# cliarie/radix-join

Measured on AMD Instinct MI355X. Metric: probe_tuples_per_sec, higher is better.
Workload: dtype int32

## Files before the change

### include/rj.h

```cpp
#ifndef RJ_H_
#define RJ_H_

#include <stddef.h>
#include <stdint.h>

#ifdef __cplusplus
extern "C" {
#endif

#define RJ_PAGE_SIZE 8192u

typedef enum rj_dtype {
    RJ_INT32   = 0,
    RJ_INT64   = 1,
    RJ_FP64    = 2,
    RJ_VARCHAR = 3
} rj_dtype;

typedef enum rj_status {
    RJ_OK            = 0,
    RJ_ERR_ARG       = 1,
    RJ_ERR_DEVICE    = 2,
    RJ_ERR_NOMEM     = 3,
    RJ_ERR_DATA      = 4,
// ... 243 lines not shown
    uint64_t bins;
} rj_partition_pass;
typedef struct rj_partition_plan {
    uint32_t passes;
    uint32_t pbits[RJ_PLAN_MAX_PASSES];
    int32_t  fine, fine_xcd;
    uint32_t fine_grid;
    int32_t  mid, last;
    int32_t  spec, spec2;
    uint64_t spec_cap_max, spec2_cap_max;
    uint64_t n_first_out, n_last_out;
    uint32_t tpg_first, reserved;
    rj_partition_pass pass[RJ_PLAN_MAX_PASSES];
} rj_partition_plan;
int rj_debug_partition_plan(const rj_partition_request* req, uint32_t compute_units, rj_partition_plan* out);
uint64_t rj_table_num_rows(const rj_table* t);
uint64_t rj_table_col_pages(const rj_table* t, uint64_t col);
int      rj_table_copy_pages(rj_context* ctx, const rj_table* t, uint64_t col, void* const* dst, uint64_t n_dst);

typedef struct rj_result rj_result;

enum { RJ_EXEC_KEEP_ON_DEVICE = 1 };

int rj_execute(rj_context* ctx, const rj_plan* plan, rj_result** out);
int rj_execute_resident(rj_context* ctx, const rj_plan* plan, rj_table* const* tables,
                        uint64_t n_tables, int32_t flags, rj_result** out);

uint64_t rj_result_num_rows(const rj_result* r);
uint64_t rj_result_num_cols(const rj_result* r);
int32_t  rj_result_col_type(const rj_result* r, uint64_t col);
// ... 58 lines not shown
```

### radix-join_amd/csrc/rj_api.hip

```cpp
#include <chrono>
#include <cstdlib>
#include <mutex>

#include "rj_frame.hpp"
#include "rj_fsum.hpp"
#include "rj_internal.hpp"
#include "rj_radix_plan.hpp"
#include "rj_sortkey.hpp"
#include "rj_xplan.hpp"

using namespace rj;

static std::mutex  g_err_mu;
static std::string g_create_error;

template <class F>
static int guarded(rj_context* ctx, F&& f) {
    try {
        f();
        return RJ_OK;
    } catch (const rj::Error& e) {
        if (ctx) ctx->last_error = e.what();
        return e.code;
    } catch (const std::bad_alloc&) {
// ... 191 lines not shown
    *n_out = 0;
    try {
        rj::map_eval_row(ops, n_ops, n_cols, col_type, col_bits, col_null, out_cap, out_bits, out_null, out_kind, n_out);
        return RJ_OK;
    } catch (const rj::Error& e) {
        std::lock_guard<std::mutex> g(g_err_mu);
        g_create_error = e.what();
        return e.code;
    } catch (const std::exception& e) {
        std::lock_guard<std::mutex> g(g_err_mu);
        g_create_error = e.what();
        return RJ_ERR_DEVICE;
    }
}

int rj_debug_partition_plan(const rj_partition_request* req, uint32_t compute_units, rj_partition_plan* out) {
    if (!req || !out) return RJ_ERR_ARG;
    if (req->key_words < 1 || req->key_words > 2 || req->carry_words < 0 || req->key_words + req->carry_words > MAX_WORDS) return RJ_ERR_ARG;
    if (req->bits > 32 || (req->single_pass && req->bits > (uint32_t)PT_MAXBITS)) return RJ_ERR_ARG;
    if (req->word_source < 0 || req->word_source > 2 || (req->word_source == 2 && (req->key_words != 1 || req->carry_words != 1))) return RJ_ERR_ARG;
    RadixFacts f;
    f.n = req->n;
    f.KW = req->key_words, f.CW = req->carry_words, f.bits = req->bits, f.shift0 = req->shift0;
    f.single_pass = req->single_pass != 0;
    f.word_src = req->word_source != 0, f.word_src_packed = req->word_source == 2;
    f.external = req->external != 0, f.composite = req->composite != 0;
    f.preseg_nseg = req->preseg_nseg, f.preseg_n_oseg = req->preseg_n_oseg;
    f.after_offsets = req->after_offsets != 0, f.spec_flag = req->flag_word != 0, f.spec2_ok = req->spec2_ok != 0;
    Tuning tune;
    tune.from_env();
    const RadixPlan pl = radix_plan(f, tune, (int)compute_units);
    static_assert((int)RadixMid::Aos3Side == RJ_MID_AOS3_SIDE && (int)RadixLast::Aos3 == RJ_LAST_AOS3 &&
                      (int)RadixOffsets::Chunked == RJ_OFF_CHUNKED && (int)RadixHist::LastSample == RJ_HIST_LAST_SAMPLE &&
                      (int)RadixScatter::LastDense == RJ_SCATTER_LAST_DENSE,
                  "include/rj.h lists the plan's enums in the order of rj_radix_plan.hpp");
    *out = rj_partition_plan{};
    out->passes = pl.passes();
    out->fine = pl.fine, out->fine_xcd = pl.fine_xcd, out->fine_grid = pl.fine_grid;
    out->mid = (int32_t)pl.mid, out->last = (int32_t)pl.last;
    out->spec = pl.spec, out->spec2 = pl.spec2;
    out->spec_cap_max = pl.spec_cap_max, out->spec2_cap_max = pl.spec2_cap_max;
    out->n_first_out = pl.n_first_out, out->n_last_out = pl.n_last_out;
    out->tpg_first = pl.tpg_first;
    for (uint32_t p = 0; p < pl.passes() && p < RJ_PLAN_MAX_PASSES; ++p) {
        const RadixPass&   ps = pl.pass[p];
        rj_partition_pass& o = out->pass[p];
        out->pbits[p] = pl.pbits[p];
        o.bits = ps.bits, o.tiles_per_group = ps.tiles_per_group, o.xcd_log2 = ps.xcd_log2, o.xcd_remap = ps.xcd_remap;
        o.nseg_in = ps.nseg_in, o.n_oseg = ps.n_oseg, o.n_groups = ps.n_groups, o.bins = ps.bins;
        o.offsets = (int32_t)ps.offsets, o.hist = (int32_t)ps.hist, o.scatter = (int32_t)ps.scatter;
    }
    return RJ_OK;
}

int rj_debug_launch_log(rj_context* ctx, int on) {
    if (!ctx) return RJ_ERR_ARG;
    for (int l = 0; l < ctx->n_lanes(); ++l) {
        ctx->lane(l)->klog.clear();
        ctx->lane(l)->klog.on = on != 0;
    }
    return RJ_OK;
}

int rj_debug_launch_read(rj_context* ctx, char* buf, uint64_t cap, uint64_t* need) {
    if (!ctx || !need || (cap && !buf)) return RJ_ERR_ARG;
    return guarded(ctx, [&] {
// ... 275 lines not shown
```

### radix-join_amd/csrc/rj_context.hip

```cpp
#include <dlfcn.h>

#include <algorithm>
#include <chrono>
#include <cstdlib>

#include "rj_internal.hpp"

namespace rj {

[[noreturn]] void launch_failed(const char* kernel, const char* what, bool unsupported) {
    throw_fmt(unsupported ? RJ_ERR_UNSUPPORTED : RJ_ERR_DEVICE, "launch %s: %s", kernel, what);
}

static int env_int(const char* name, int def) {
    const char* v = getenv(name);
    return v && *v ? atoi(v) : def;
}

void Tuning::from_env() {
    blocked_mid = env_int("RJ_TUNE_BLOCKED_MID", blocked_mid);
    mall_chunk = env_int("RJ_TUNE_MALL_CHUNK", mall_chunk);
    radix_bits = env_int("RJ_TUNE_RADIX_BITS", radix_bits);
    p1_bits = env_int("RJ_TUNE_P1_BITS", p1_bits);
    fine = env_int("RJ_TUNE_FINE", fine);
// ... 1 lines not shown
    aos3 = env_int("RJ_TUNE_AOS3", aos3);
    aos_mid = env_int("RJ_TUNE_AOS_MID", aos_mid);
    tpg1 = env_int("RJ_TUNE_TPG1", tpg1);
    xcd_split = env_int("RJ_TUNE_XCD_SPLIT", xcd_split);
    tpg2 = env_int("RJ_TUNE_TPG2", tpg2);
    packed_side = env_int("RJ_TUNE_PACKED_SIDE", packed_side);
    xcd_min_rows = env_int("RJ_TUNE_XCD_MIN_ROWS", xcd_min_rows);
    spec_p1 = env_int("RJ_TUNE_SPEC_P1", spec_p1);
    spec_min_rows = env_int("RJ_TUNE_SPEC_MIN_ROWS", spec_min_rows);
    spec_sample = std::min(5, std::max(1, env_int("RJ_TUNE_SPEC_SAMPLE", spec_sample)));
    spec_z = std::max(0, env_int("RJ_TUNE_SPEC_Z", spec_z));
    spec_p2 = env_int("RJ_TUNE_SPEC_P2", spec_p2);
    spec2_min_rows = env_int("RJ_TUNE_SPEC2_MIN_ROWS", spec2_min_rows);
    spec2_sample = std::min(4, std::max(1, env_int("RJ_TUNE_SPEC2_SAMPLE", spec2_sample)));
    spec2_z = std::max(0, env_int("RJ_TUNE_SPEC2_Z", spec2_z));
    bcast = env_int("RJ_TUNE_BCAST", bcast);
    diag = env_int("RJ_DIAG", diag);
    varchar_dev_rows = env_int("RJ_TUNE_VARCHAR_DEV", varchar_dev_rows);
    vkey_hash_bits = env_int("RJ_DEBUG_VKEY_HASH_BITS", vkey_hash_bits);
    sync_upload = env_int("RJ_SYNC_UPLOAD", sync_upload);
    wide_carry = env_int("RJ_TUNE_WIDE_CARRY", wide_carry);
    fold_owner = env_int("RJ_TUNE_FOLD_OWNER", fold_owner);
    group_grid = env_int("RJ_TUNE_GROUP_GRID", group_grid);
    win_grid = env_int("RJ_TUNE_WIN_GRID", win_grid);
    map_grid = env_int("RJ_TUNE_MAP_GRID", map_grid);
    setop_grid = env_int("RJ_TUNE_SETOP_GRID", setop_grid);
    exchange_timeout_ms = env_int("RJ_EXCHANGE_TIMEOUT_MS", exchange_timeout_ms);
    bringup_timeout_ms = env_int("RJ_BRINGUP_TIMEOUT_MS", bringup_timeout_ms);
    debug_shard_fail = env_int("RJ_DEBUG_SHARD_FAIL", debug_shard_fail);
    debug_shard_fail_rank = env_int("RJ_DEBUG_SHARD_FAIL_RANK", debug_shard_fail_rank);
// ... 299 lines not shown
```

### radix-join_amd/csrc/rj_exec.hip

```cpp
#include <algorithm>
#include <chrono>
#include <cmath>
#include <cstdlib>
#include <functional>
#include <set>
#include <tuple>

#include "rj_expr.hpp"
#include "rj_internal.hpp"
#include "rj_radix.hpp"
#include "rj_xplan.hpp"

namespace rj {

const NodeKind* node_kind(int kind) {
    static const NodeKind kinds[] = {
        {RJ_NODE_SCAN, "a scan", "RJ_NODE_SCAN", 0, true},
        {RJ_NODE_JOIN, "a join", "RJ_NODE_JOIN", 2, true},
        {RJ_NODE_SEMI, "a semi join", "RJ_NODE_SEMI", 2, false},
        {RJ_NODE_ANTI, "an anti join", "RJ_NODE_ANTI", 2, false},
        {RJ_NODE_OUTER, "an outer join", "RJ_NODE_OUTER", 2, false},
        {RJ_NODE_FULL, "a full outer join", "RJ_NODE_FULL", 2, false},
        {RJ_NODE_AGG, "an aggregation", "RJ_NODE_AGG", 1, false},
        {RJ_NODE_SELECT, "a selection", "RJ_NODE_SELECT", 1, false},
// ... 584 lines not shown
    }

    struct CoParts {
        Parted   B, P;
        BufP     tasks;
        uint32_t max_tasks = 0;
    };
    CoParts partition_sides(JoinState& st, const JoinSpec& js, uint32_t bits, const BufP* counters = nullptr, bool spec2_ok = false) {
        CoParts        cp;
        const TupleSrc sb = make_src(st, st.bs(), js), sp = make_src(st, st.ps(), js);
        uint32_t*      fl = counters ? (*counters)->as<uint32_t>() + 4 : nullptr;
        PartitionRequest rb = PartitionRequest::columns(sb, st.KW, st.bs().CW, bits), rp = PartitionRequest::columns(sp, st.KW, st.ps().CW, bits);
        rb.spec_flag = fl;
        rp.spec_flag = fl ? fl + 1 : nullptr;
        rb.spec2_ok = rp.spec2_ok = spec2_ok;
        cp.B = partition(rb);
        cp.P = partition(rp);
        return cp;
    }
    int  spec_fallbacks = 0;
    void repartition_exact(JoinState& st, const JoinSpec& js, uint32_t bits, CoParts& cp, const BufP& counters, bool flag_b,
                           bool flag_p) {
        ++spec_fallbacks;
        if (ctx->tune.diag >= 1)
            fprintf(stderr, "[rj diag] %s: a speculative pass overflowed (build side %d, probe side %d): exact partition again (fallback %d of this plan)\n",
                    st.kind->name, (int)flag_b, (int)flag_p, spec_fallbacks);
        if (flag_b) {
            const TupleSrc sb = make_src(st, st.bs(), js);
            cp.B = Parted();
            cp.B = partition(PartitionRequest::columns(sb, st.KW, st.bs().CW, bits));
        }
        if (flag_p) {
// ... 2445 lines not shown
```

### radix-join_amd/csrc/rj_internal.hpp

```cpp
#pragma once
#include <hip/hip_runtime.h>

#include <atomic>
#include <cstdarg>
#include <cstdio>
#include <cstring>
#include <functional>
#include <map>
#include <memory>
#include <mutex>
#include <stdexcept>
#include <string>
#include <vector>

#include "../../include/rj.h"
#include "rj_comm.hpp"
#include "rj_device.hpp"
#include "rj_kernels.hpp"

namespace rj {

struct Context;

struct Error : std::runtime_error {
// ... 153 lines not shown
    int aos3 = 1;
    int aos_mid = 2;
    int tpg1 = 0;
    int packed_side = 0;
    int tpg2 = 0;
    int xcd_min_rows = 40 << 20;
    int xcd_split = 1;
    int spec_p1 = 1;
    int spec_min_rows = 40 << 20;
    int spec_sample = 5;
    int spec_z = 60;
    int spec_p2 = 1;
    int spec2_min_rows = 40 << 20;
    int spec2_sample = 2;
    int spec2_z = 70;
    int bcast = 1;
    int diag = 0;
    int varchar_dev_rows = 200000;
    int vkey_hash_bits = 0;
    int sync_upload = 0;
    int wide_carry = 1;
    int fold_owner = 1;
    int group_grid = 0;
    int map_grid = 0;
    int win_grid = 0;
    int setop_grid = 0;
    int exchange_timeout_ms = 120000;
    int bringup_timeout_ms = 0;
    int debug_shard_fail = 0, debug_shard_fail_rank = 0;
    int debug_poison = 0;
// ... 129 lines not shown
```

### radix-join_amd/csrc/rj_radix.hip

```cpp
#include "rj_radix.hpp"

#include <algorithm>

#include "rj_radix_plan.hpp"

namespace rj {

void read_back(Context* ctx, void* dst, const void* src, size_t bytes) {
    try {
        RJ_HIP(hipMemcpyAsync(dst, src, bytes, hipMemcpyDeviceToHost, ctx->stream));
        ctx->sync();
    } catch (...) {
        (void)hipStreamSynchronize(ctx->stream);
        throw;
    }
}

namespace {

RadixFacts facts_of(const PartitionRequest& rq) {
    RadixFacts f;
    f.n = rq.ws ? rq.ws->n : (rq.src ? rq.src->n_rows : 0);
    f.KW = rq.KW, f.CW = rq.CW, f.bits = rq.bits, f.shift0 = rq.shift0, f.single_pass = rq.single_pass;
    f.word_src = rq.ws != nullptr, f.word_src_packed = rq.ws && rq.ws->packed;
// ... 36 lines not shown
    PassParams       pp{};
    SpecParams       sp{};
    LastParams       lp{};
    BufP             grp_start, off, hist, cursor;
    const uint32_t*  in_end = nullptr;
    const uint32_t*  oseg_base = nullptr;
    PassRun(const RadixPass& s, uint32_t pass) : ps(s), p(pass), F(1u << s.bits) {}
};

class Driver {
   public:
    Driver(Context* c, const Launch& l, const PartitionRequest& r)
        : ctx(c), L(l), rq(r), src(r.src ? *r.src : none), n(r.ws ? r.ws->n : src.n_rows),
          pl(radix_plan(facts_of(r), c->tune, c->compute_units())), passes(pl.passes()) {}

    Parted run() {
        P.NW = rq.KW + rq.CW;
        P.packed = pl.packed(), P.aos3 = pl.aos3(), P.spec = pl.spec, P.spec2 = pl.spec2;
        allocate();
        shift = rq.shift0;
        cur = rq.ws ? rq.ws->w : Words{};
        nxt = (pl.aos3() && passes == 1) ? waos : wa;
        for (uint32_t p = 0; p < passes; ++p) {
            PassRun r(pl.pass[p], p);
            begin_pass(r);
            offsets_for_pass(r);
            if (p == 0 && rq.after_offsets) (*rq.after_offsets)(r.off->as<uint32_t>());
            if (p == 0 && pl.chunk_second()) send_sizes_to_host(r);
            if (r.ps.offsets != RadixOffsets::Chunked) scatter_pass(r);
            advance(r);
        }
        P.w = cur;
        for (int a = 0; a < P.NW; ++a) P.wbuf[a] = cur_is_a ? A[a] : B[a];
        if (pl.aos3()) P.wbuf[0] = AOS;
        P.off = seg_off;
        P.NP = nseg;
        P.pbits = pl.pbits;
        const PassShape* shape = rq.shape;
        if (shape && !shape->prior_bits.empty()) P.pbits.insert(P.pbits.begin(), shape->prior_bits.begin(), shape->prior_bits.end());
        P.n_tuples = n;
        return std::move(P);
    }

   private:
    Context*                ctx;
    const Launch&           L;
    const PartitionRequest& rq;
    const TupleSrc          none{};
    const TupleSrc&         src;
    const uint64_t          n;
    const RadixPlan         pl;
    const uint32_t          passes;
    Parted                  P;
    BufP  A[MAX_WORDS], B[MAX_WORDS], AOS, MID[2], SIDE[2];
    Words wa{}, wb{}, waos{};
    BufP  fine_off, fine_cursor, coarse_off, coarse_cursor;
    BufP  last_limit, last_seg_sum, last_grp;
    BufP  spec_start, spec_limit, spec_end;
    Event chunk_ev;
    BufP     seg_off;
    uint32_t nseg = 1, shift = 0;
    Words    cur{}, nxt{};
    bool     cur_is_a = false;

    void allocate() {
        const uint32_t mids = std::min<uint32_t>(passes - 1, 2);
        if (pl.aos_mid())
            for (uint32_t k = 0; k < mids; ++k) {
                MID[k] = ctx->buf(std::max<uint64_t>(n, 1) * 12);
                if (pl.mid == RadixMid::Aos3Side) SIDE[k] = ctx->buf(std::max<uint64_t>(n, 1) * 2 + 16);
            }
        if (pl.mid == RadixMid::PackedSide)
            for (uint32_t k = 0; k < mids; ++k) SIDE[k] = ctx->buf(std::max<uint64_t>(n, 1) * 2 + 16);
        if (pl.aos3()) {
            AOS = ctx->buf(std::max<uint64_t>(pl.n_last_out, 1) * 12);
            waos.w[0] = AOS->as<uint32_t>();
        }
        for (int a = 0; a < (pl.packed() ? 1 : P.NW); ++a) {
            if (pl.pair_word >= 0 && a == pl.pair_word + 1) continue;
            const uint64_t wbytes = (pl.packed() || a == pl.pair_word) ? 8 : 4;
            if (rq.external) {
                wa.w[a] = rq.external->w[a];
                continue;
            }
            if ((pl.aos3() && passes == 1) || pl.aos_mid()) continue;
            A[a] = ctx->buf(pl.n_first_out * wbytes + 2048);
            wa.w[a] = A[a]->as<uint32_t>();
            if (passes > (pl.aos3() ? 2u : 1u)) {
                B[a] = ctx->buf(pl.n_last_out * wbytes + 2048);
                wb.w[a] = B[a]->as<uint32_t>();
            }
        }
    }

    void begin_pass(PassRun& r) {
        const RadixPass& ps = r.ps;
        const PassShape* shape = r.p == 0 ? rq.shape : nullptr;
        const bool       preseg = shape && shape->nseg > 0;
        PassParams&      pp = r.pp;
        pp.nseg = nseg;
        pp.n = (uint32_t)n;
        pp.shift = shift;
        pp.fanout_log2 = ps.bits;
        pp.tiles_per_group = ps.tiles_per_group;
        pp.xcd_log2 = ps.xcd_log2;
        pp.xcd_remap = ps.xcd_remap;
        if (shape && shape->hi_shift) {
            pp.hi_shift = shape->hi_shift;
            pp.lo_bits = shape->lo_bits;
        }
        r.in_end = preseg ? shape->seg_end : (ps.spec_in ? spec_end->as<uint32_t>() : nullptr);
        r.oseg_base = preseg ? shape->oseg_off : (seg_off ? seg_off->as<uint32_t>() : nullptr);
        if (r.p == 0 && !preseg) return;
        const uint32_t* in_off = preseg ? shape->seg_begin : (ps.spec_in ? spec_start->as<uint32_t>() : seg_off->as<uint32_t>());
        r.grp_start = ctx->buf(((uint64_t)ps.nseg_in + 1) * 4);
        launch_group_table(L, in_off, ps.nseg_in, ps.tiles_per_group * (uint32_t)PT_TILE, r.grp_start->as<uint32_t>(), r.in_end);
        pp.nseg = ps.nseg_in;
        pp.seg_off = in_off;
        pp.seg_end = r.in_end;
        pp.oseg_shift = preseg ? shape->oseg_shift : (ps.spec_in ? 3u : 0u);
        pp.grp_start = r.grp_start->as<uint32_t>();
    }

    void offsets_for_pass(PassRun& r) {
        switch (r.ps.offsets) {
        case RadixOffsets::Fine:
            if (r.ps.hist != RadixHist::None) fine_histogram();
            r.off = r.p == 0 ? coarse_off : fine_off;
            r.cursor = r.p == 0 ? coarse_cursor : fine_cursor;
            r.pp.cursor = r.cursor->as<uint32_t>();
// ... 55 lines not shown
        const uint32_t G = r.ps.n_groups, prev = (r.p + 1) % 2;
        switch (r.ps.hist) {
        case RadixHist::Src: launch_pass_hist_src(L, src, rq.KW, r.pp, G); break;
        case RadixHist::Digits: launch_pass_hist_digits(L, SIDE[prev]->as<uint16_t>(), r.pp, G); break;
        case RadixHist::Aos3: launch_pass_hist_aos3(L, MID[prev]->as<uint32_t>(), r.pp, G); break;
        case RadixHist::Blocked: launch_pass_hist_blocked(L, cur.w[0], r.pp, G); break;
        case RadixHist::Packed: launch_pass_hist_packed(L, cur.w[0], r.pp, G); break;
        case RadixHist::Dense: launch_pass_hist_dense(L, cur, r.pp, G); break;
        default: throw_fmt(RJ_ERR_DEVICE, "radix plan: pass %u has no exact histogram", r.p);
        }
    }

    void sample_first(PassRun& r) {
        const uint32_t spec_s = (uint32_t)ctx->tune.spec_sample;
        const uint32_t nb = (uint32_t)r.ps.bins << 3;
        r.hist = ctx->buf((uint64_t)nb * 4);
        r.off = ctx->buf((r.ps.bins + 1) * 4);
        r.cursor = ctx->buf((uint64_t)nb * 8);
        spec_start = ctx->buf((uint64_t)nb * 4);
        spec_limit = ctx->buf((uint64_t)nb * 4);
        spec_end = ctx->buf((uint64_t)nb * 4);
        RJ_HIP(hipMemsetAsync(r.hist->p, 0, (uint64_t)nb * 4, ctx->stream));
        r.pp.hist = r.hist->as<uint32_t>();
        r.sp.cursor = r.cursor->as<unsigned long long>();
        r.sp.flag = rq.spec_flag;
        r.sp.sink = (uint32_t)pl.spec_cap_max;
        r.sp.sample_log2 = spec_s;
        launch_pass_sample_src(L, src, rq.KW, r.pp, r.sp, r.ps.n_groups);
        launch_spec_caps(L, r.pp.hist, nb, spec_s, (float)(ctx->tune.spec_z / 10.0), (uint32_t)pl.spec_cap_max,
                         spec_start->as<uint32_t>(), spec_limit->as<uint32_t>(), r.sp.cursor);
    }

    void sample_last(PassRun& r) {
        const uint32_t spec2_s = (uint32_t)ctx->tune.spec2_sample;
        const uint32_t nb = (uint32_t)r.ps.bins, nseg_in = r.ps.nseg_in;
        r.hist = ctx->buf((uint64_t)nb * 4);
        r.off = ctx->buf((uint64_t)nb * 8);
        r.cursor = ctx->buf((uint64_t)nb * 4);
        last_limit = ctx->buf((uint64_t)nb * 4);
        last_seg_sum = ctx->buf((uint64_t)r.ps.n_oseg * 8);
        RJ_HIP(hipMemsetAsync(r.hist->p, 0, (uint64_t)nb * 4, ctx->stream));
        r.pp.hist = r.hist->as<uint32_t>();
        r.lp.cursor32 = r.cursor->as<uint32_t>();
        r.lp.limit = last_limit->as<uint32_t>();
        r.lp.flag = rq.spec_flag;
        r.lp.sink = (uint32_t)pl.spec2_cap_max;
        r.lp.sample_log2 = spec2_s;
        PassParams ps = r.pp;
        ps.tiles_per_group = LAST_SAMPLE_TPG;
        last_grp = ctx->buf(((uint64_t)nseg_in + 1) * 4);
        launch_group_table(L, r.pp.seg_off, nseg_in, LAST_SAMPLE_TPG * (uint32_t)PT_TILE, last_grp->as<uint32_t>(), r.in_end);
        ps.grp_start = last_grp->as<uint32_t>();
        launch_last_sample(L, cur.w[0], P.packed, ps, r.lp, r.ps.sample_groups);
        launch_last_caps(L, r.pp.hist, r.ps.n_oseg, r.F, spec2_s, (float)(ctx->tune.spec2_z / 10.0), (uint32_t)pl.spec2_cap_max,
                         last_seg_sum->as<unsigned long long>(), r.off->as<uint32_t>(), last_limit->as<uint32_t>(), r.lp.cursor32);
    }

    void send_sizes_to_host(PassRun& r) {
        const uint64_t bytes = (r.ps.bins + 1) * 4;
        if (bytes > Context::SMALL_PINNED / 4) throw_fmt(RJ_ERR_DEVICE, "chunked pass: too many segments");
        RJ_HIP(hipMemcpyAsync(ctx->small_pinned(), r.off->p, bytes, hipMemcpyDeviceToHost, ctx->stream));
        chunk_ev.make();
        RJ_HIP(hipEventRecord(chunk_ev.e, ctx->stream));
    }

// ... 47 lines not shown
            pp.side_out = SIDE[p % 2]->as<uint16_t>();
            pp.next_shift = shift + ps.bits;
            pp.next_mask = (1u << pl.pbits[p + 1]) - 1u;
        }
        const SpecParams* sp = (p == 0 && pl.spec) ? &r.sp : nullptr;
        switch (ps.scatter) {
        case RadixScatter::Src: launch_pass_scatter_src(L, src, rq.KW, rq.CW, pp, G, nxt, ps.aos_out, sp); break;
        case RadixScatter::SrcPacked: launch_pass_scatter_src_packed(L, src, pp, G, nxt.w[0], ps.blocked_out, sp); break;
        case RadixScatter::Dense: launch_pass_scatter_dense(L, cur, P.NW, pl.pair_word, pp, G, nxt, ps.aos_out); break;
        case RadixScatter::Packed: launch_pass_scatter_packed(L, cur.w[0], pp, G, nxt.w[0]); break;
        case RadixScatter::Blocked: launch_pass_scatter_blocked(L, cur.w[0], pp, G, nxt.w[0], ps.blocked_out); break;
        case RadixScatter::Aos3: launch_pass_scatter_aos3(L, MID[(p + 1) % 2]->as<uint32_t>(), pp, G, nxt.w[0]); break;
        case RadixScatter::LastBlocked: launch_last_scatter_blocked(L, cur.w[0], pp, G, nxt.w[0], r.lp); break;
        case RadixScatter::LastDense: launch_last_scatter_dense(L, cur, pp, G, nxt, r.lp); break;
        }
        const uint32_t bins = (uint32_t)ps.bins;
        if (ps.hist == RadixHist::LastSample) {
            launch_last_close(L, r.lp.cursor32, last_limit->as<uint32_t>(), bins, r.off->as<uint32_t>());
            if (ctx->tune.diag >= 1) spec_report(ctx, r.cursor, last_limit, r.off, bins, n, pl.n_last_out, 2);
            P.off_shift = 1;
        }
        if (ps.hist == RadixHist::SampleSrc) {
            launch_spec_close(L, r.sp.cursor, spec_start->as<uint32_t>(), spec_limit->as<uint32_t>(), r.F, spec_end->as<uint32_t>(),
                              r.off->as<uint32_t>());
            if (ctx->tune.diag >= 1) spec_report(ctx, r.cursor, spec_limit, spec_start, bins << 3, n, pl.n_first_out, 1);
        }
    }

    void advance(PassRun& r) {
        seg_off = r.off;
        nseg = (uint32_t)r.ps.bins;
        shift += r.ps.bits;
        cur = nxt;
        cur_is_a = (r.p % 2 == 0);
        nxt = cur_is_a ? wb : wa;
        if (pl.aos3() && r.p + 2 == passes) nxt = waos;
    }
};

}

Parted radix_partition(Context* ctx, const Launch& L, const PartitionRequest& rq) { return Driver(ctx, L, rq).run(); }

}
```

### radix-join_amd/csrc/rj_radix.hpp

```cpp
#pragma once
#include <functional>

#include "rj_internal.hpp"

namespace rj {

struct Parted {
    int      NW = 0;
    BufP     wbuf[MAX_WORDS];
    Words    w{};
    BufP     off;
    uint32_t NP = 0;
    std::vector<uint32_t> pbits;
    bool     packed = false;
    bool     aos3 = false;
    uint64_t n_tuples = 0;
    bool     spec = false;
    uint32_t off_shift = 0;
    bool     spec2 = false;
};

struct WordSrc {
    Words    w{};
    uint64_t n = 0;
// ... 26 lines not shown

    static PartitionRequest columns(const TupleSrc& s, int KW, int CW, uint32_t bits) {
        PartitionRequest rq;
        rq.src = &s, rq.KW = KW, rq.CW = CW, rq.bits = bits;
        return rq;
    }
    static PartitionRequest words(const WordSrc& s, int KW, int CW, uint32_t bits) {
        PartitionRequest rq;
        rq.ws = &s, rq.KW = KW, rq.CW = CW, rq.bits = bits;
        return rq;
    }
};

Parted radix_partition(Context* ctx, const Launch& L, const PartitionRequest& rq);

struct Event {
    hipEvent_t e = nullptr;
    Event() = default;
    Event(const Event&) = delete;
    Event& operator=(const Event&) = delete;
    void make() { RJ_HIP(hipEventCreateWithFlags(&e, hipEventDisableTiming)); }
    ~Event() {
        if (e) (void)hipEventDestroy(e);
    }
};

void read_back(Context* ctx, void* dst, const void* src, size_t bytes);

}
```

### radix-join_amd/csrc/rj_radix_plan.cpp

```cpp
#include "rj_radix_plan.hpp"

#include <algorithm>
#include <cmath>

#include "rj_internal.hpp"

namespace rj {

uint32_t radix_tiles_per_group(uint64_t tuples_per_segment, uint64_t target_groups) {
    uint64_t k = (tuples_per_segment + (uint64_t)PT_TILE * target_groups - 1) / ((uint64_t)PT_TILE * target_groups);
    return (uint32_t)std::min<uint64_t>(std::max<uint64_t>(k, 1), 8);
}

uint64_t radix_cap_bound(double B, double C, uint32_t s, double z) {
    const double bound = std::ldexp(C + z * std::sqrt(B * (C + B)) + 0.5 * z * z * B, (int)s) + 32.0 * B;
    return bound < 4.0e9 ? (((uint64_t)std::ceil(bound) + 255u) & ~(uint64_t)255u) : ~(uint64_t)0 >> 1;
}

namespace {

void choose_layout(const RadixFacts& f, const Tuning& t, int compute_units, RadixPlan& pl) {
    const uint64_t n = f.n;
    const uint32_t passes = pl.passes(), bits = f.bits;
    const bool     shaped = f.composite || f.preseg_nseg > 0;
// ... 112 lines not shown
        if (b1 < f.bits && b1 <= PT_CAPBITS && f.bits - b1 <= PT_CAPBITS) {
            pl.pbits[0] = b1;
            pl.pbits[1] = f.bits - b1;
        }
    }
    pl.pass.resize(passes);
    choose_layout(f, t, compute_units, pl);
    uint32_t nseg = 1;
    for (uint32_t p = 0; p < passes; ++p) {
        plan_pass(f, t, pl, p, nseg, pl.pass[p]);
        nseg = (uint32_t)pl.pass[p].bins;
    }
    return pl;
}

}
```

### radix-join_amd/csrc/rj_radix_plan.hpp

```cpp
#pragma once
#include <cstdint>
#include <vector>

namespace rj {

struct Tuning;

struct RadixFacts {
    uint64_t n = 0;
    int      KW = 1, CW = 0;
    uint32_t bits = 0, shift0 = 0;
    bool     single_pass = false;
    bool     word_src = false, word_src_packed = false;
    bool     external = false;
    bool     composite = false;
    uint32_t preseg_nseg = 0, preseg_n_oseg = 0;
    bool     after_offsets = false;
    bool     spec_flag = false, spec2_ok = false;
};

enum class RadixMid : int32_t {
    Dense = 0,
    Packed = 1,
    PackedSide = 2,
// ... 41 lines not shown
    bool packed() const { return last == RadixLast::Packed; }
    bool aos3() const { return last == RadixLast::Aos3; }
    bool aos_mid() const { return mid == RadixMid::Aos3 || mid == RadixMid::Aos3Side; }
    bool side() const { return mid == RadixMid::Aos3Side || mid == RadixMid::PackedSide; }
    bool chunk_second() const { return pass.size() == 2 && pass[1].offsets == RadixOffsets::Chunked; }
};

constexpr uint32_t LAST_SAMPLE_TPG = 8;

uint32_t radix_tiles_per_group(uint64_t tuples_per_segment, uint64_t target_groups);

uint64_t radix_cap_bound(double B, double C, uint32_t s, double z);

RadixPlan radix_plan(const RadixFacts& f, const Tuning& tune, int compute_units);

}
```

### radix-join_amd/pyrj/capi.py

```python
from __future__ import annotations

import ctypes as C
import os

import numpy as np

from . import pages as pg
from . import plan as pl

PKG_DIR = os.path.dirname(os.path.dirname(os.path.abspath(__file__)))
LIB_PATH = os.path.join(PKG_DIR, "librj.so")

RJ_EXEC_KEEP_ON_DEVICE = 1


class rj_comm_id(C.Structure):
    _fields_ = [("bytes", C.c_char * 128)]


class rj_config(C.Structure):
    _fields_ = [
        ("device", C.c_int32),
        ("profile", C.c_int32),
        ("stream", C.c_void_p),
# ... 115 lines not shown
    "rj_comm_id_create",
    "rj_execute_sharded",
    "rj_plan_shardable",
    "rj_table_upload",
    "rj_table_adopt_device",
    "rj_table_release",
    "rj_table_from_csv",
    "rj_debug_parse_fp64",
    "rj_debug_sort_key",
    "rj_debug_sort_key_value",
    "rj_debug_win_frame",
    "rj_debug_win_ntile",
    "rj_debug_fsum",
    "rj_debug_map_eval",
    "rj_debug_partition_plan",
    "rj_table_num_rows",
    "rj_table_col_pages",
    "rj_table_copy_pages",
    "rj_execute",
    "rj_execute_resident",
    "rj_result_num_rows",
    "rj_result_num_cols",
    "rj_result_col_type",
    "rj_result_col_pages",
    "rj_result_copy_pages",
    "rj_result_device_pages",
    "rj_result_free",
    "rj_exchange_plan",
    "rj_shard_partition",
    "rj_join_tuples",
# ... 521 lines not shown
                ("reserved", C.c_uint32), ("pass_", rj_partition_pass * 4)]


PLAN_MID = ["dense", "packed", "packed_side", "blocked", "aos3", "aos3_side"]
PLAN_LAST = ["dense", "packed", "aos3"]
PLAN_OFFSETS = ["fine", "hist", "sample", "chunked"]
PLAN_HIST = ["none", "fine_src", "fine_words", "src", "digits", "aos3", "blocked", "packed", "dense", "sample_src", "last_sample"]
PLAN_SCATTER = ["src", "src_packed", "dense", "packed", "blocked", "aos3", "last_blocked", "last_dense"]


def partition_plan(n, kw=1, cw=1, bits=0, *, cus=256, shift0=0, single_pass=False, word_source=0, external=False, composite=False,
                   preseg=(0, 0), after_offsets=False, flag_word=False, spec2_ok=False) -> dict:
    L = load()
    L.rj_debug_partition_plan.restype = C.c_int
    L.rj_debug_partition_plan.argtypes = [C.POINTER(rj_partition_request), C.c_uint32, C.POINTER(rj_partition_plan)]
    rq = rj_partition_request(int(n), kw, cw, bits, shift0, int(single_pass), int(word_source), int(external), int(composite),
                              preseg[0], preseg[1], int(after_offsets), int(flag_word), int(spec2_ok))
    out = rj_partition_plan()
    rc = L.rj_debug_partition_plan(C.byref(rq), cus, C.byref(out))
    if rc != 0:
        raise RjError(rc, "rj_debug_partition_plan: bad request")
    d = {k: int(getattr(out, k)) for k in ("passes", "fine_grid", "spec_cap_max", "spec2_cap_max", "n_first_out", "n_last_out", "tpg_first")}
    d.update({k: bool(getattr(out, k)) for k in ("fine", "fine_xcd", "spec", "spec2")})
    d["pbits"] = [int(out.pbits[p]) for p in range(d["passes"])]
    d["mid"], d["last"] = PLAN_MID[out.mid], PLAN_LAST[out.last]
    d["pass"] = []
    for p in range(d["passes"]):
        ps = out.pass_[p]
        e = {k: int(getattr(ps, k)) for k in ("bits", "tiles_per_group", "xcd_log2", "xcd_remap", "nseg_in", "n_oseg", "n_groups", "bins")}
        e["offsets"], e["hist"], e["scatter"] = PLAN_OFFSETS[ps.offsets], PLAN_HIST[ps.hist], PLAN_SCATTER[ps.scatter]
        d["pass"].append(e)
    return d


def make_comm_id() -> bytes:
    L = load()
    preload_torch_rccl()
    cid = rj_comm_id()
    rc = L.rj_comm_id_create(C.byref(cid))
    if rc != 0:
        raise RjError(rc, (L.rj_last_error(None) or b"").decode())
    return C.string_at(C.addressof(cid), 128)


def build_context(**kw):
    return Context(**kw)


def destroy_context(ctx: Context):
# ... 6 lines not shown
```

Measured before the change: 35.04 billion.

## Interleave build and probe radix partition passes across two streams

```diff
diff --git a/include/rj.h b/include/rj.h
--- a/include/rj.h
+++ b/include/rj.h
@@ -281,6 +281,19 @@
     rj_partition_pass pass[RJ_PLAN_MAX_PASSES];
 } rj_partition_plan;
 int rj_debug_partition_plan(const rj_partition_request* req, uint32_t compute_units, rj_partition_plan* out);
+typedef enum rj_lane_kind { RJ_LANE_OFFSETS = 0, RJ_LANE_SCATTER = 1, RJ_LANE_CLOSE = 2, RJ_LANE_JOIN = 3 } rj_lane_kind;
+typedef struct rj_lane_step {
+    int32_t  side;
+    uint32_t pass;
+    int32_t  kind;
+    int32_t  lane;
+} rj_lane_step;
+typedef struct rj_lane_edge {
+    uint32_t after, before;
+} rj_lane_edge;
+int rj_debug_lane_schedule(const rj_partition_request* build, const rj_partition_request* probe, uint32_t compute_units,
+                           int32_t mask, rj_lane_step* steps, uint64_t step_cap, uint64_t* n_steps, rj_lane_edge* edges,
+                           uint64_t edge_cap, uint64_t* n_edges);
 uint64_t rj_table_num_rows(const rj_table* t);
 uint64_t rj_table_col_pages(const rj_table* t, uint64_t col);
 int      rj_table_copy_pages(rj_context* ctx, const rj_table* t, uint64_t col, void* const* dst, uint64_t n_dst);
diff --git a/radix-join_amd/csrc/rj_api.hip b/radix-join_amd/csrc/rj_api.hip
--- a/radix-join_amd/csrc/rj_api.hip
+++ b/radix-join_amd/csrc/rj_api.hip
@@ -229,12 +229,11 @@
     }
 }
 
-int rj_debug_partition_plan(const rj_partition_request* req, uint32_t compute_units, rj_partition_plan* out) {
-    if (!req || !out) return RJ_ERR_ARG;
-    if (req->key_words < 1 || req->key_words > 2 || req->carry_words < 0 || req->key_words + req->carry_words > MAX_WORDS) return RJ_ERR_ARG;
-    if (req->bits > 32 || (req->single_pass && req->bits > (uint32_t)PT_MAXBITS)) return RJ_ERR_ARG;
-    if (req->word_source < 0 || req->word_source > 2 || (req->word_source == 2 && (req->key_words != 1 || req->carry_words != 1))) return RJ_ERR_ARG;
-    RadixFacts f;
+static bool facts_of_request(const rj_partition_request* req, RadixFacts& f) {
+    if (!req) return false;
+    if (req->key_words < 1 || req->key_words > 2 || req->carry_words < 0 || req->key_words + req->carry_words > MAX_WORDS) return false;
+    if (req->bits > 32 || (req->single_pass && req->bits > (uint32_t)PT_MAXBITS)) return false;
+    if (req->word_source < 0 || req->word_source > 2 || (req->word_source == 2 && (req->key_words != 1 || req->carry_words != 1))) return false;
     f.n = req->n;
     f.KW = req->key_words, f.CW = req->carry_words, f.bits = req->bits, f.shift0 = req->shift0;
     f.single_pass = req->single_pass != 0;
@@ -242,6 +241,12 @@
     f.external = req->external != 0, f.composite = req->composite != 0;
     f.preseg_nseg = req->preseg_nseg, f.preseg_n_oseg = req->preseg_n_oseg;
     f.after_offsets = req->after_offsets != 0, f.spec_flag = req->flag_word != 0, f.spec2_ok = req->spec2_ok != 0;
+    return true;
+}
+
+int rj_debug_partition_plan(const rj_partition_request* req, uint32_t compute_units, rj_partition_plan* out) {
+    RadixFacts f;
+    if (!out || !facts_of_request(req, f)) return RJ_ERR_ARG;
     Tuning tune;
     tune.from_env();
     const RadixPlan pl = radix_plan(f, tune, (int)compute_units);
@@ -265,6 +270,24 @@
         o.nseg_in = ps.nseg_in, o.n_oseg = ps.n_oseg, o.n_groups = ps.n_groups, o.bins = ps.bins;
         o.offsets = (int32_t)ps.offsets, o.hist = (int32_t)ps.hist, o.scatter = (int32_t)ps.scatter;
     }
+    return RJ_OK;
+}
+
+int rj_debug_lane_schedule(const rj_partition_request* build, const rj_partition_request* probe, uint32_t compute_units, int32_t mask,
+                           rj_lane_step* steps, uint64_t step_cap, uint64_t* n_steps, rj_lane_edge* edges, uint64_t edge_cap,
+                           uint64_t* n_edges) {
+    RadixFacts fb, fp;
+    if (!n_steps || !n_edges || (step_cap && !steps) || (edge_cap && !edges)) return RJ_ERR_ARG;
+    if (!facts_of_request(build, fb) || !facts_of_request(probe, fp)) return RJ_ERR_ARG;
+    static_assert((int)LaneKind::Join == RJ_LANE_JOIN, "include/rj.h lists the lane kinds in the order of rj_radix_plan.hpp");
+    Tuning tune;
+    tune.from_env();
+    const LaneSchedule S = lane_schedule(radix_plan(fb, tune, (int)compute_units), radix_plan(fp, tune, (int)compute_units),
+                                         mask < 0 ? tune.lanes : mask);
+    *n_steps = S.steps.size(), *n_edges = S.edges.size();
+    for (size_t i = 0; i < S.steps.size() && i < step_cap; ++i)
+        steps[i] = rj_lane_step{S.steps[i].side, S.steps[i].pass, (int32_t)S.steps[i].kind, S.steps[i].lane};
+    for (size_t i = 0; i < S.edges.size() && i < edge_cap; ++i) edges[i] = rj_lane_edge{S.edges[i].after, S.edges[i].before};
     return RJ_OK;
 }
 
diff --git a/radix-join_amd/csrc/rj_context.hip b/radix-join_amd/csrc/rj_context.hip
--- a/radix-join_amd/csrc/rj_context.hip
+++ b/radix-join_amd/csrc/rj_context.hip
@@ -39,6 +39,7 @@
     spec2_min_rows = env_int("RJ_TUNE_SPEC2_MIN_ROWS", spec2_min_rows);
     spec2_sample = std::min(4, std::max(1, env_int("RJ_TUNE_SPEC2_SAMPLE", spec2_sample)));
     spec2_z = std::max(0, env_int("RJ_TUNE_SPEC2_Z", spec2_z));
+    lanes = env_int("RJ_TUNE_LANES", lanes) & 3;
     bcast = env_int("RJ_TUNE_BCAST", bcast);
     diag = env_int("RJ_DIAG", diag);
     varchar_dev_rows = env_int("RJ_TUNE_VARCHAR_DEV", varchar_dev_rows);
diff --git a/radix-join_amd/csrc/rj_exec.hip b/radix-join_amd/csrc/rj_exec.hip
--- a/radix-join_amd/csrc/rj_exec.hip
+++ b/radix-join_amd/csrc/rj_exec.hip
@@ -622,8 +622,9 @@
         rb.spec_flag = fl;
         rp.spec_flag = fl ? fl + 1 : nullptr;
         rb.spec2_ok = rp.spec2_ok = spec2_ok;
-        cp.B = partition(rb);
-        cp.P = partition(rp);
+        std::pair<Parted, Parted> bp = radix_partition_pair(ctx, L, rb, rp);
+        cp.B = std::move(bp.first);
+        cp.P = std::move(bp.second);
         return cp;
     }
     int  spec_fallbacks = 0;
diff --git a/radix-join_amd/csrc/rj_internal.hpp b/radix-join_amd/csrc/rj_internal.hpp
--- a/radix-join_amd/csrc/rj_internal.hpp
+++ b/radix-join_amd/csrc/rj_internal.hpp
@@ -191,6 +191,7 @@
     int spec2_min_rows = 40 << 20;
     int spec2_sample = 2;
     int spec2_z = 70;
+    int lanes = 0;
     int bcast = 1;
     int diag = 0;
     int varchar_dev_rows = 200000;
diff --git a/radix-join_amd/csrc/rj_radix.hip b/radix-join_amd/csrc/rj_radix.hip
--- a/radix-join_amd/csrc/rj_radix.hip
+++ b/radix-join_amd/csrc/rj_radix.hip
@@ -74,22 +74,56 @@
         : ctx(c), L(l), rq(r), src(r.src ? *r.src : none), n(r.ws ? r.ws->n : src.n_rows),
           pl(radix_plan(facts_of(r), c->tune, c->compute_units())), passes(pl.passes()) {}
 
+    const RadixPlan& plan() const { return pl; }
+
     Parted run() {
+        start(false);
+        for (uint32_t p = 0; p < passes; ++p) {
+            offsets(p, L.stream);
+            scatter(p, L.stream);
+            close(p, L.stream);
+        }
+        return finish();
+    }
+
+    void start(bool hold_passes) {
+        hold = hold_passes;
         P.NW = rq.KW + rq.CW;
         P.packed = pl.packed(), P.aos3 = pl.aos3(), P.spec = pl.spec, P.spec2 = pl.spec2;
         allocate();
         shift = rq.shift0;
         cur = rq.ws ? rq.ws->w : Words{};
         nxt = (pl.aos3() && passes == 1) ? waos : wa;
-        for (uint32_t p = 0; p < passes; ++p) {
-            PassRun r(pl.pass[p], p);
-            begin_pass(r);
-            offsets_for_pass(r);
-            if (p == 0 && rq.after_offsets) (*rq.after_offsets)(r.off->as<uint32_t>());
-            if (p == 0 && pl.chunk_second()) send_sizes_to_host(r);
-            if (r.ps.offsets != RadixOffsets::Chunked) scatter_pass(r);
-            advance(r);
-        }
+        runs.resize(passes);
+        if (hold)
+            for (uint32_t p = 0; p < passes; ++p) reserve(p);
+    }
+
+    void offsets(uint32_t p, hipStream_t s) {
+        L.stream = s;
+        if (!runs[p]) reserve(p);
+        PassRun& r = *runs[p];
+        begin_pass(r);
+        offsets_for_pass(r);
+        if (p == 0 && rq.after_offsets) (*rq.after_offsets)(r.off->as<uint32_t>());
+        if (p == 0 && pl.chunk_second()) send_sizes_to_host(r);
+    }
+
+    void scatter(uint32_t p, hipStream_t s) {
+        L.stream = s;
+        PassRun& r = *runs[p];
+        if (r.ps.offsets != RadixOffsets::Chunked) scatter_pass(r);
+    }
+
+    void close(uint32_t p, hipStream_t s) {
+        L.stream = s;
+        PassRun& r = *runs[p];
+        close_pass(r);
+        advance(r);
+        if (!hold) runs[p].reset();
+    }
+
+    Parted finish() {
         P.w = cur;
         for (int a = 0; a < P.NW; ++a) P.wbuf[a] = cur_is_a ? A[a] : B[a];
         if (pl.aos3()) P.wbuf[0] = AOS;
@@ -104,7 +138,7 @@
 
    private:
     Context*                ctx;
-    const Launch&           L;
+    Launch                  L;
     const PartitionRequest& rq;
     const TupleSrc          none{};
     const TupleSrc&         src;
@@ -122,6 +156,8 @@
     uint32_t nseg = 1, shift = 0;
     Words    cur{}, nxt{};
     bool     cur_is_a = false;
+    bool     hold = false;
+    std::vector<std::unique_ptr<PassRun>> runs;
 
     void allocate() {
         const uint32_t mids = std::min<uint32_t>(passes - 1, 2);
@@ -150,6 +186,32 @@
                 B[a] = ctx->buf(pl.n_last_out * wbytes + 2048);
                 wb.w[a] = B[a]->as<uint32_t>();
             }
+        }
+    }
+
+    void reserve(uint32_t p) {
+        runs[p].reset(new PassRun(pl.pass[p], p));
+        PassRun&         r = *runs[p];
+        const RadixPass& ps = r.ps;
+        const bool       preseg = p == 0 && rq.shape && rq.shape->nseg > 0;
+        if (p > 0 || preseg) r.grp_start = ctx->buf(((uint64_t)ps.nseg_in + 1) * 4);
+        if (ps.offsets != RadixOffsets::Sample) return;
+        if (ps.hist == RadixHist::SampleSrc) {
+            const uint32_t nb = (uint32_t)ps.bins << 3;
+            r.hist = ctx->buf((uint64_t)nb * 4);
+            r.off = ctx->buf((ps.bins + 1) * 4);
+            r.cursor = ctx->buf((uint64_t)nb * 8);
+            spec_start = ctx->buf((uint64_t)nb * 4);
+            spec_limit = ctx->buf((uint64_t)nb * 4);
+            spec_end = ctx->buf((uint64_t)nb * 4);
+        } else {
+            const uint32_t nb = (uint32_t)ps.bins;
+            r.hist = ctx->buf((uint64_t)nb * 4);
+            r.off = ctx->buf((uint64_t)nb * 8);
+            r.cursor = ctx->buf((uint64_t)nb * 4);
+            last_limit = ctx->buf((uint64_t)nb * 4);
+            last_seg_sum = ctx->buf((uint64_t)ps.n_oseg * 8);
+            last_grp = ctx->buf(((uint64_t)ps.nseg_in + 1) * 4);
         }
     }
 
@@ -173,7 +235,6 @@
         r.oseg_base = preseg ? shape->oseg_off : (seg_off ? seg_off->as<uint32_t>() : nullptr);
         if (r.p == 0 && !preseg) return;
         const uint32_t* in_off = preseg ? shape->seg_begin : (ps.spec_in ? spec_start->as<uint32_t>() : seg_off->as<uint32_t>());
-        r.grp_start = ctx->buf(((uint64_t)ps.nseg_in + 1) * 4);
         launch_group_table(L, in_off, ps.nseg_in, ps.tiles_per_group * (uint32_t)PT_TILE, r.grp_start->as<uint32_t>(), r.in_end);
         pp.nseg = ps.nseg_in;
         pp.seg_off = in_off;
@@ -259,13 +320,7 @@
     void sample_first(PassRun& r) {
         const uint32_t spec_s = (uint32_t)ctx->tune.spec_sample;
         const uint32_t nb = (uint32_t)r.ps.bins << 3;
-        r.hist = ctx->buf((uint64_t)nb * 4);
-        r.off = ctx->buf((r.ps.bins + 1) * 4);
-        r.cursor = ctx->buf((uint64_t)nb * 8);
-        spec_start = ctx->buf((uint64_t)nb * 4);
-        spec_limit = ctx->buf((uint64_t)nb * 4);
-        spec_end = ctx->buf((uint64_t)nb * 4);
-        RJ_HIP(hipMemsetAsync(r.hist->p, 0, (uint64_t)nb * 4, ctx->stream));
+        RJ_HIP(hipMemsetAsync(r.hist->p, 0, (uint64_t)nb * 4, L.stream));
         r.pp.hist = r.hist->as<uint32_t>();
         r.sp.cursor = r.cursor->as<unsigned long long>();
         r.sp.flag = rq.spec_flag;
@@ -279,12 +334,7 @@
     void sample_last(PassRun& r) {
         const uint32_t spec2_s = (uint32_t)ctx->tune.spec2_sample;
         const uint32_t nb = (uint32_t)r.ps.bins, nseg_in = r.ps.nseg_in;
-        r.hist = ctx->buf((uint64_t)nb * 4);
-        r.off = ctx->buf((uint64_t)nb * 8);
-        r.cursor = ctx->buf((uint64_t)nb * 4);
-        last_limit = ctx->buf((uint64_t)nb * 4);
-        last_seg_sum = ctx->buf((uint64_t)r.ps.n_oseg * 8);
-        RJ_HIP(hipMemsetAsync(r.hist->p, 0, (uint64_t)nb * 4, ctx->stream));
+        RJ_HIP(hipMemsetAsync(r.hist->p, 0, (uint64_t)nb * 4, L.stream));
         r.pp.hist = r.hist->as<uint32_t>();
         r.lp.cursor32 = r.cursor->as<uint32_t>();
         r.lp.limit = last_limit->as<uint32_t>();
@@ -293,7 +343,6 @@
         r.lp.sample_log2 = spec2_s;
         PassParams ps = r.pp;
         ps.tiles_per_group = LAST_SAMPLE_TPG;
-        last_grp = ctx->buf(((uint64_t)nseg_in + 1) * 4);
         launch_group_table(L, r.pp.seg_off, nseg_in, LAST_SAMPLE_TPG * (uint32_t)PT_TILE, last_grp->as<uint32_t>(), r.in_end);
         ps.grp_start = last_grp->as<uint32_t>();
         launch_last_sample(L, cur.w[0], P.packed, ps, r.lp, r.ps.sample_groups);
@@ -371,17 +420,22 @@
         case RadixScatter::LastBlocked: launch_last_scatter_blocked(L, cur.w[0], pp, G, nxt.w[0], r.lp); break;
         case RadixScatter::LastDense: launch_last_scatter_dense(L, cur, pp, G, nxt, r.lp); break;
         }
-        const uint32_t bins = (uint32_t)ps.bins;
+    }
+
+    void close_pass(PassRun& r) {
+        const RadixPass& ps = r.ps;
+        const uint32_t   bins = (uint32_t)ps.bins;
+        const bool       report = ctx->tune.diag >= 1 && ps.offsets == RadixOffsets::Sample;
         if (ps.hist == RadixHist::LastSample) {
             launch_last_close(L, r.lp.cursor32, last_limit->as<uint32_t>(), bins, r.off->as<uint32_t>());
-            if (ctx->tune.diag >= 1) spec_report(ctx, r.cursor, last_limit, r.off, bins, n, pl.n_last_out, 2);
             P.off_shift = 1;
         }
-        if (ps.hist == RadixHist::SampleSrc) {
+        if (ps.hist == RadixHist::SampleSrc)
             launch_spec_close(L, r.sp.cursor, spec_start->as<uint32_t>(), spec_limit->as<uint32_t>(), r.F, spec_end->as<uint32_t>(),
                               r.off->as<uint32_t>());
-            if (ctx->tune.diag >= 1) spec_report(ctx, r.cursor, spec_limit, spec_start, bins << 3, n, pl.n_first_out, 1);
-        }
+        if (report && L.stream != ctx->stream) RJ_HIP(hipStreamSynchronize(L.stream));
+        if (report && ps.hist == RadixHist::LastSample) spec_report(ctx, r.cursor, last_limit, r.off, bins, n, pl.n_last_out, 2);
+        if (report && ps.hist == RadixHist::SampleSrc) spec_report(ctx, r.cursor, spec_limit, spec_start, bins << 3, n, pl.n_first_out, 1);
     }
 
     void advance(PassRun& r) {
@@ -399,4 +453,56 @@
 
 Parted radix_partition(Context* ctx, const Launch& L, const PartitionRequest& rq) { return Driver(ctx, L, rq).run(); }
 
+std::pair<Parted, Parted> radix_partition_pair(Context* ctx, const Launch& L, const PartitionRequest& rqB, const PartitionRequest& rqP) {
+    {
+        const int cus = ctx->compute_units();
+        if (!radix_plan(facts_of(rqB), ctx->tune, cus).spec && !radix_plan(facts_of(rqP), ctx->tune, cus).spec) {
+            Parted b = radix_partition(ctx, L, rqB);
+            Parted p = radix_partition(ctx, L, rqP);
+            return {std::move(b), std::move(p)};
+        }
+    }
+    Driver             B(ctx, L, rqB), P(ctx, L, rqP);
+    Driver* const      side[2] = {&B, &P};
+    const LaneSchedule S = lane_schedule(B.plan(), P.plan(), ctx->tune.lanes);
+    bool               two = false;
+    for (const LaneStep& st : S.steps) two |= st.lane != 0;
+    B.start(true);
+    P.start(true);
+    const hipStream_t  lane[2] = {L.stream, two ? ctx->aux_stream() : L.stream};
+    Event              fork;
+    std::vector<Event> done(S.steps.size());
+    try {
+        if (two) {
+            fork.make();
+            RJ_HIP(hipEventRecord(fork.e, lane[0]));
+            RJ_HIP(hipStreamWaitEvent(lane[1], fork.e, 0));
+        }
+        for (uint32_t i = 0; i < (uint32_t)S.steps.size(); ++i) {
+            const LaneStep&   st = S.steps[i];
+            const hipStream_t s = lane[st.lane];
+            bool              record = false;
+            for (const LaneEdge& e : S.edges) {
+                if (e.before == i) RJ_HIP(hipStreamWaitEvent(s, done[e.after].e, 0));
+                record |= e.after == i;
+            }
+            switch (st.kind) {
+            case LaneKind::Offsets: side[st.side]->offsets(st.pass, s); break;
+            case LaneKind::Scatter: side[st.side]->scatter(st.pass, s); break;
+            case LaneKind::Close: side[st.side]->close(st.pass, s); break;
+            case LaneKind::Join: break;
+            }
+            if (record) {
+                done[i].make();
+                RJ_HIP(hipEventRecord(done[i].e, s));
+            }
+        }
+    } catch (...) {
+        if (two) (void)hipStreamSynchronize(lane[1]);
+        throw;
+    }
+    Parted b = B.finish(), p = P.finish();
+    return {std::move(b), std::move(p)};
 }
+
+}
diff --git a/radix-join_amd/csrc/rj_radix.hpp b/radix-join_amd/csrc/rj_radix.hpp
--- a/radix-join_amd/csrc/rj_radix.hpp
+++ b/radix-join_amd/csrc/rj_radix.hpp
@@ -64,6 +64,9 @@
 
 Parted radix_partition(Context* ctx, const Launch& L, const PartitionRequest& rq);
 
+std::pair<Parted, Parted> radix_partition_pair(Context* ctx, const Launch& L, const PartitionRequest& build,
+                                               const PartitionRequest& probe);
+
 struct Event {
     hipEvent_t e = nullptr;
     Event() = default;
diff --git a/radix-join_amd/csrc/rj_radix_plan.cpp b/radix-join_amd/csrc/rj_radix_plan.cpp
--- a/radix-join_amd/csrc/rj_radix_plan.cpp
+++ b/radix-join_amd/csrc/rj_radix_plan.cpp
@@ -150,4 +150,49 @@
     return pl;
 }
 
+LaneSchedule lane_schedule(const RadixPlan& build, const RadixPlan& probe, int mask) {
+    const RadixPlan* pl[2] = {&build, &probe};
+    if (build.chunk_second() || probe.chunk_second()) mask = 0;
+    LaneSchedule S;
+    std::vector<int> at[2];
+    for (int s = 0; s < 2; ++s) at[s].assign((size_t)pl[s]->passes() * 3, -1);
+    auto slot = [&](int s, uint32_t p, LaneKind k) -> int& { return at[s][(size_t)p * 3 + (size_t)k]; };
+    auto sampled = [&](int s, uint32_t p) { return pl[s]->pass[p].offsets == RadixOffsets::Sample; };
+    auto emit = [&](int s, uint32_t p, LaneKind k, bool aux) {
+        int need = -1;
+        if (k == LaneKind::Offsets && p > 0) need = slot(s, p - 1, LaneKind::Close);
+        if (k == LaneKind::Scatter) need = slot(s, p, LaneKind::Offsets);
+        if (k == LaneKind::Close) need = slot(s, p, LaneKind::Scatter);
+        const uint32_t me = (uint32_t)S.steps.size();
+        if (need >= 0 && S.steps[(size_t)need].lane != (aux ? 1 : 0)) S.edges.push_back({(uint32_t)need, me});
+        S.steps.push_back({s, p, k, aux ? 1 : 0});
+        slot(s, p, k) = (int)me;
+    };
+    const uint32_t deepest = std::max(build.passes(), probe.passes());
+    for (uint32_t p = 0; p < deepest; ++p)
+        for (int s = 0; s < 2; ++s) {
+            if (p >= pl[s]->passes()) continue;
+            if (p > 0 && slot(s, p - 1, LaneKind::Close) < 0) emit(s, p - 1, LaneKind::Close, false);
+            if (slot(s, p, LaneKind::Offsets) < 0) emit(s, p, LaneKind::Offsets, false);
+            for (int s2 = 0; s2 < 2; ++s2)
+                for (uint32_t p2 = 0; p2 < pl[s2]->passes(); ++p2) {
+                    if (!sampled(s2, p2)) continue;
+                    if (slot(s2, p2, LaneKind::Offsets) < 0 && (p2 == 0 || slot(s2, p2 - 1, LaneKind::Close) >= 0))
+                        emit(s2, p2, LaneKind::Offsets, (mask & (p2 == 0 ? LANES_FIRST_OFFSETS : LANES_LAST)) != 0);
+                    if (slot(s2, p2, LaneKind::Scatter) >= 0 && slot(s2, p2, LaneKind::Close) < 0)
+                        emit(s2, p2, LaneKind::Close, (mask & LANES_LAST) != 0);
+                }
+            emit(s, p, LaneKind::Scatter, false);
+        }
+    for (uint32_t p = 0; p < deepest; ++p)
+        for (int s = 0; s < 2; ++s)
+            if (p < pl[s]->passes() && slot(s, p, LaneKind::Close) < 0) emit(s, p, LaneKind::Close, false);
+    int last_aux = -1;
+    for (size_t i = 0; i < S.steps.size(); ++i)
+        if (S.steps[i].lane == 1) last_aux = (int)i;
+    if (last_aux >= 0) S.edges.push_back({(uint32_t)last_aux, (uint32_t)S.steps.size()});
+    S.steps.push_back({-1, 0, LaneKind::Join, 0});
+    return S;
 }
+
+}
diff --git a/radix-join_amd/csrc/rj_radix_plan.hpp b/radix-join_amd/csrc/rj_radix_plan.hpp
--- a/radix-join_amd/csrc/rj_radix_plan.hpp
+++ b/radix-join_amd/csrc/rj_radix_plan.hpp
@@ -79,4 +79,27 @@
 
 RadixPlan radix_plan(const RadixFacts& f, const Tuning& tune, int compute_units);
 
+enum class LaneKind : int32_t {
+    Offsets = 0,
+    Scatter = 1,
+    Close = 2,
+    Join = 3,
+};
+struct LaneStep {
+    int32_t  side = 0;
+    uint32_t pass = 0;
+    LaneKind kind = LaneKind::Offsets;
+    int32_t  lane = 0;
+};
+struct LaneEdge {
+    uint32_t after = 0, before = 0;
+};
+struct LaneSchedule {
+    std::vector<LaneStep> steps;
+    std::vector<LaneEdge> edges;
+};
+constexpr int LANES_FIRST_OFFSETS = 1;
+constexpr int LANES_LAST = 2;
+LaneSchedule lane_schedule(const RadixPlan& build, const RadixPlan& probe, int mask);
+
 }
diff --git a/radix-join_amd/pyrj/capi.py b/radix-join_amd/pyrj/capi.py
--- a/radix-join_amd/pyrj/capi.py
+++ b/radix-join_amd/pyrj/capi.py
@@ -153,6 +153,7 @@
     "rj_debug_fsum",
     "rj_debug_map_eval",
     "rj_debug_partition_plan",
+    "rj_debug_lane_schedule",
     "rj_table_num_rows",
     "rj_table_col_pages",
     "rj_table_copy_pages",
@@ -704,8 +705,8 @@
     L = load()
     L.rj_debug_partition_plan.restype = C.c_int
     L.rj_debug_partition_plan.argtypes = [C.POINTER(rj_partition_request), C.c_uint32, C.POINTER(rj_partition_plan)]
-    rq = rj_partition_request(int(n), kw, cw, bits, shift0, int(single_pass), int(word_source), int(external), int(composite),
-                              preseg[0], preseg[1], int(after_offsets), int(flag_word), int(spec2_ok))
+    rq = _partition_request(n, kw, cw, bits, shift0=shift0, single_pass=single_pass, word_source=word_source, external=external,
+                            composite=composite, preseg=preseg, after_offsets=after_offsets, flag_word=flag_word, spec2_ok=spec2_ok)
     out = rj_partition_plan()
     rc = L.rj_debug_partition_plan(C.byref(rq), cus, C.byref(out))
     if rc != 0:
@@ -723,6 +724,42 @@
     return d
 
 
+def _partition_request(n, kw=1, cw=1, bits=0, *, shift0=0, single_pass=False, word_source=0, external=False, composite=False,
+                       preseg=(0, 0), after_offsets=False, flag_word=False, spec2_ok=False):
+    return rj_partition_request(int(n), kw, cw, bits, shift0, int(single_pass), int(word_source), int(external), int(composite),
+                                preseg[0], preseg[1], int(after_offsets), int(flag_word), int(spec2_ok))
+
+
+class rj_lane_step(C.Structure):
+    _fields_ = [("side", C.c_int32), ("pass_", C.c_uint32), ("kind", C.c_int32), ("lane", C.c_int32)]
+
+
+class rj_lane_edge(C.Structure):
+    _fields_ = [("after", C.c_uint32), ("before", C.c_uint32)]
+
+
+LANE_KIND = ["offsets", "scatter", "close", "join"]
+LANE = ["main", "aux"]
+
+
+def lane_schedule(build: dict, probe: dict, *, mask=-1, cus=256):
+    L = load()
+    L.rj_debug_lane_schedule.restype = C.c_int
+    L.rj_debug_lane_schedule.argtypes = [C.POINTER(rj_partition_request), C.POINTER(rj_partition_request), C.c_uint32, C.c_int32,
+                                         C.POINTER(rj_lane_step), C.c_uint64, C.POINTER(C.c_uint64), C.POINTER(rj_lane_edge),
+                                         C.c_uint64, C.POINTER(C.c_uint64)]
+    rb, rp = _partition_request(**build), _partition_request(**probe)
+    cap = 64
+    steps, edges = (rj_lane_step * cap)(), (rj_lane_edge * cap)()
+    ns, ne = C.c_uint64(0), C.c_uint64(0)
+    rc = L.rj_debug_lane_schedule(C.byref(rb), C.byref(rp), cus, mask, steps, cap, C.byref(ns), edges, cap, C.byref(ne))
+    if rc != 0 or ns.value > cap or ne.value > cap:
+        raise RjError(rc, "rj_debug_lane_schedule: bad request")
+    out = [{"side": {0: "B", 1: "P"}.get(steps[i].side), "pass": int(steps[i].pass_), "kind": LANE_KIND[steps[i].kind],
+            "lane": LANE[steps[i].lane]} for i in range(ns.value)]
+    return out, [(int(edges[i].after), int(edges[i].before)) for i in range(ne.value)]
+
+
 def make_comm_id() -> bytes:
     L = load()
     preload_torch_rccl()
```

New measurement: 35.01 billion. About the same (-0.1%).
